# qiyueyao/Kubernetes-verification

Measured on AMD Instinct MI355X. Metric: pod-pairs/sec for reachability build + all-checks latency, 100k pods, 1/2/4/8 GPU, higher is better.
Workload: dtype u64

## Files before the change

include/kano_hip.h:

```cpp
#ifndef KANO_HIP_H
#define KANO_HIP_H

#include <stddef.h>
#include <stdint.h>

#ifdef __cplusplus
extern "C" {
#endif

typedef struct kano_ctx kano_ctx;

#define KANO_PATH_AUTO    0
#define KANO_PATH_BITWISE 1
#define KANO_PATH_MFMA    2

#define KANO_INFO_N        0
#define KANO_INFO_W        1
#define KANO_INFO_P        2
#define KANO_INFO_U        3
#define KANO_INFO_NNZ_SEL  4
#define KANO_INFO_NNZ_ALW  5
#define KANO_INFO_HEAVY    6
#define KANO_INFO_ROW0     7
#define KANO_INFO_ROW1     8
#define KANO_INFO_MAXSEL   9
#define KANO_INFO_UA      10
#define KANO_INFO_HEAVY_PATH 11
#define KANO_INFO_WORK_ITEMS 12
#define KANO_INFO_ROWS_KERNEL 13
#define KANO_INFO_ROWS_CUS 14
#define KANO_INFO_HEAVY_SEL 15
#define KANO_INFO_HEAVY_KERNEL 16
#define KANO_INFO_CLS_REUSED 17
#define KANO_INFO_NSLOTS   18

int  kano_create(int device, kano_ctx** out);
int  kano_create_lean(int device, kano_ctx** out);
void kano_destroy(kano_ctx* ctx);
const char* kano_last_error(const kano_ctx* ctx);
int  kano_set_stream(kano_ctx* ctx, void* hip_stream);

int kano_set_pods(kano_ctx* ctx, int64_t n, int32_t ncols, const int32_t* pod_val);
int kano_set_policies(kano_ctx* ctx, int64_t P,
                      const int64_t* sel_off, const int32_t* sel_col, const int32_t* sel_val,
                      const int64_t* alw_off, const int32_t* alw_col, const int32_t* alw_val);
int kano_set_shard(kano_ctx* ctx, int64_t row_begin, int64_t row_end);

int kano_build(kano_ctx* ctx, int path);
int kano_info(kano_ctx* ctx, int64_t* out );
// ... 182 lines not shown
```

kubernetes-verification_amd/csrc/kano_engine.hpp:

```cpp
#pragma once
#include <hip/hip_runtime.h>
#include <hip/hip_ext.h>

#include <algorithm>
#include <cmath>
#include <functional>
#include <cerrno>
#include <cstdint>
#include <cstdlib>
#include <cstring>
#include <string>
#include <vector>
#include <array>
#include <chrono>
#include <ctime>
#include <cstdio>
#include <dlfcn.h>
#include <link.h>
#include <thread>

#include "kano_hip.h"
#include "kano_internal.hpp"
#include "kano_prims.hpp"

// ... 26 lines not shown
  DBuf keys_d, table, smin, slot_of, flag, cid, cls, rep, mcnt, mcur, moff, mem, cval;
};

struct RowsInputs {
  DBuf wioff, wicls, soffc, slist, aloff, alist, alcoff, alc, rmoff, rmem, cmoff, cmem, ccls,
      hflag, hlist, Mc;
};

struct SideMatch {
  i64 nterms = 0;
  int NM = 0;
  bool dense = false;
  DBuf toff, tslot, tval, pmask, moff, mslot;
  DBuf table, pslot, gcnt, goff, gcur, gmem, pstart, plen, bits, bcnt, boff;
  i64 T = 0;
};

enum {
  SZ_UR = 0, SZ_UA, SZ_NNZ_SEL, SZ_NNZ_ALC, SZ_NNZ_ALW, SZ_NFLAGS, SZ_WI, SZ_HEAVY, SZ_MAXSEL,
  SZ_LIGHT, SZ_HSEL, SZ_NL, SZ_PAIRS, SZ_IDX0, SZ_IDX1, SZ_IDX2, SZ_IDX3, SZ_ERR, SZ_SLOTS = 18,
  SZ_SIGNAL = SZ_SLOTS
};

constexpr size_t ROW_STAGE_BYTES = 256 * 1024;

struct kano_ctx {
  int device = 0;
  hipStream_t stream = nullptr;
  bool own_stream = false;
  std::string err;
// ... 63 lines not shown
  bool xcd_tried = false, eng_on_xcd = false, xcd_last_ok = false;
  int side_mode = 0;
  int xcd_side = -1;
  hipStream_t stream_x = nullptr, stream2_x = nullptr, stream3x = nullptr;
  hipStream_t stream2_u = nullptr;
  hipEvent_t ev_sw = nullptr, ev_sw2 = nullptr;
  i64 rows_cu_bytes = 8ll << 30;
  int num_cus = 0, rows_cus = 0;

  ClassSet rc, cc;
  bool cls_valid = false;
  bool cls_reuse = false;
  i64 cls_U[2] = {0, 0};
  i64 cls_reused = 0;
  SideMatch sm, am;
  i64 UAW = 0, ldC = 0;
  i64 nnz_sel = 0, nnz_alc = 0, nnz_alw = 0, heavy_count = 0, wi_total = 0, nflags = 0;
  i64 heavy_sel = 0;
  i64 light_cost = 0;
  bool rows_use_alist = false;
  int max_sel = 0;
  int heavy_path = 0;
  int heavy_kernel = 0;
  int rows_kernel = 0;

  DBuf pv;
  DBuf scnt, cost, soffc, scur, slist, ecls, wicls, maxs, wicnt, wioff, hflag, hoff, hlist, sq, pfoff;
  DBuf ACT, AC, nca, acnt, alcoff, alc, aloff, alist;
  DBuf M, Mc, color, colnand, col_and, col_or_c, col_nand_c;
  DBuf scan_tmp;
// ... 157 lines not shown
struct GroupRun {
  int32_t group;
  int32_t first, len;
};
i64 group_chunks(const kano_ctx* ctx);
i64 group_run_rows(kano_ctx* ctx, i64 sel, i64 nbp, bool rows);
int group_masks_launch(kano_ctx* ctx, const int32_t* gd, i64 b0, i64 nbp, u64* maskT);
int group_rows_launch(kano_ctx* ctx, const u64* maskT, i64 b0, i64 nbp, const int32_t* order,
                      const GroupRun* runs, i64 nruns, i64 Gd, u64* counts, int32_t* row_counts);

template <typename T>
T* P_(DBuf& b) {
  return reinterpret_cast<T*>(b.p);
}

inline unsigned nblk(i64 n, i64 per = TPB) { return (unsigned)((n + per - 1) / per); }

}
```

kubernetes-verification_amd/csrc/kano_ext.hip:

```cpp
#include "kano_engine.hpp"
#include "kano_inc.hpp"
#include "kano_k8s.hpp"
#include "kano_path.hpp"
#include "kano_hops.hpp"

using namespace kano_eng;

namespace {

struct PathGeom {
  bool identity = false;
  i64 rows = 0;
  i64 Ua = 0;
  i64 KW = 0;
  i64 ldR = 0;
  const u64* base = nullptr;
  const u64* T = nullptr;
};

template <int CW>
int path_or_launch(kano_ctx* ctx, const u64* D, u64* R, u64* Dn, const PathGeom& g) {
  const i64 nch = (g.ldR + 64 * CW - 1) / (64 * CW);
  hipLaunchKernelGGL(k_path_or<CW>, dim3(nblk(g.rows * nch, TPB / 64)), dim3(TPB), 0, ctx->stream,
                     D, R, Dn, g.ldR, g.T, g.ldR, g.rows, g.KW, nch, P_<u64>(ctx->pcnt));
// ... 354 lines not shown
      return fail(ctx, -EINVAL, "kano_add_policies: allow term column out of range");
  if (ncols_x > 0 && n > 0) {
    const i64 have = ctx->inc_xcols * n, add = (i64)ncols_x * n;
    DBuf grown;
    KTRY(dalloc(ctx, grown, sizeof(int32_t) * (have + add)));
    if (have > 0)
      KCHK(hipMemcpyAsync(grown.p, ctx->xv.p, sizeof(int32_t) * have, hipMemcpyDeviceToDevice,
                          ctx->stream));
    KCHK(hipMemcpyAsync(P_<int32_t>(grown) + have, xval, sizeof(int32_t) * add,
                        hipMemcpyHostToDevice, ctx->stream));
    KTRY(sync(ctx));
    dfree(ctx->xv);
    ctx->xv = grown;
  }
  ctx->inc_xcols += ncols_x;
  if (ncols_x > 0) ctx->cls_valid = false;
  const i64 A0 = ctx->inc_A, A1 = A0 + Pn;
  if (A1 > ctx->inc_acap) {
    const i64 cap = std::max<i64>(A1, 2 * ctx->inc_acap);
    DBuf s2, a2;
    KTRY(dalloc(ctx, s2, sizeof(u64) * std::max<i64>(1, cap * W)));
    KTRY(dalloc(ctx, a2, sizeof(u64) * std::max<i64>(1, cap * W)));
    if (A0 > 0 && W > 0) {
      KCHK(hipMemcpyAsync(s2.p, ctx->asel.p, sizeof(u64) * A0 * W, hipMemcpyDeviceToDevice,
                          ctx->stream));
      KCHK(hipMemcpyAsync(a2.p, ctx->aalw.p, sizeof(u64) * A0 * W, hipMemcpyDeviceToDevice,
                          ctx->stream));
    }
    KTRY(sync(ctx));
    dfree(ctx->asel);
    dfree(ctx->aalw);
// ... 912 lines not shown
```

kubernetes-verification_amd/csrc/kano_hip.hip:

```cpp
#include "kano_engine.hpp"
#include "kano_kernels.hpp"

namespace kano_eng {

int fail(kano_ctx* ctx, int code, const std::string& msg) {
  ctx->err = msg;
  return code;
}

int settle(kano_ctx* ctx);

int dalloc(kano_ctx* ctx, DBuf& b, size_t bytes) {
  if (bytes == 0) bytes = 16;
  if (b.p && b.bytes >= bytes) return 0;
  if (b.p) {
    KTRY(settle(ctx));
    KCHK(hipFree(b.p));
    b.p = nullptr;
    b.bytes = 0;
  }
  const hipError_t e = hipMalloc(&b.p, bytes);
  if (e != hipSuccess) {
    b.p = nullptr;
    return fail(ctx, -ENOMEM, "hipMalloc(" + std::to_string(bytes) + " bytes) -> " +
// ... 248 lines not shown

void ring_bell(kano_ctx* ctx) {
  if (ctx->bell) __atomic_store_n(ctx->bell, ctx->bell_seq, __ATOMIC_SEQ_CST);
}

int unprime(kano_ctx* ctx) {
  if (!ctx->primed || ctx->priming) return 0;
  ctx->primed = false;
  ring_bell(ctx);
  ctx->gate_forced = ctx->bell_seq;
  KCHK(hipStreamSynchronize(ctx->stream));
  KCHK(hipStreamSynchronize(ctx->stream2));
  std::swap(ctx->sizes, ctx->sizes_alt);
  swap_rows_ptrs(ctx, !ctx->prime_kept);
  ctx->alist_valid = ctx->prime_alist_valid;
  return 0;
}

int sync(kano_ctx* ctx) {
  KTRY(unprime(ctx));
  KCHK(hipStreamSynchronize(ctx->stream));
  return 0;
}

int settle(kano_ctx* ctx) {
  KTRY(unprime(ctx));
  if (!ctx->async_pending) return 0;
  ctx->async_pending = false;
  KCHK(hipSetDevice(ctx->device));
  KCHK(hipStreamSynchronize(ctx->stream3));
// ... 270 lines not shown
  return 0;
}

int match_alloc(kano_ctx* ctx, SideMatch& sx, ClassSet& cs, FillBatch& fb) {
  const i64 P = ctx->P, U = cs.U;
  KTRY(dalloc(ctx, sx.pstart, sizeof(i64) * std::max<i64>(1, P)));
  KTRY(dalloc(ctx, sx.plen, sizeof(int32_t) * std::max<i64>(1, P)));
  if (P == 0) return 0;
  if (U == 0) {
    KTRY(fb.add(sx.pstart, sizeof(i64) * P, 0u));
    KTRY(fb.add(sx.plen, sizeof(int32_t) * P, 0u));
    return 0;
  }
  if (sx.dense) return 0;
  const int NM = sx.NM;
  sx.T = table_size(U);
  const i64 NT = std::max<i64>(1, (i64)NM * sx.T);
  KTRY(dalloc(ctx, sx.table, sizeof(int32_t) * NT));
  KTRY(dalloc(ctx, sx.pslot, sizeof(int32_t) * std::max<i64>(1, (i64)NM * U)));
  KTRY(dalloc(ctx, sx.gcnt, sizeof(int32_t) * NT));
  KTRY(dalloc(ctx, sx.gcur, sizeof(int32_t) * std::max<i64>(1, (i64)NM * U)));
  KTRY(dalloc(ctx, sx.goff, sizeof(int32_t) * (NT + 1)));
  KTRY(dalloc(ctx, sx.gmem, sizeof(int32_t) * ((i64)NM * U + U)));
  if (NM > 0) {
    KTRY(fb.add(sx.table, sizeof(int32_t) * NT, 0xffffffffu));
    KTRY(fb.add(sx.gcnt, sizeof(int32_t) * NT, 0u));
  }
  return 0;
}

// ... 5 lines not shown
  a.mslot = P_<int32_t>(sx.mslot);
  a.table = P_<int32_t>(sx.table);
  a.T = sx.T;
  a.pslot = P_<int32_t>(sx.pslot);
  a.gcnt = P_<int32_t>(sx.gcnt);
  a.goff = P_<int32_t>(sx.goff);
  a.gcur = P_<int32_t>(sx.gcur);
  a.gmem = P_<int32_t>(sx.gmem);
  a.toff = P_<i64>(sx.toff);
  a.tval = P_<int32_t>(sx.tval);
  a.pmask = P_<int32_t>(sx.pmask);
  a.pstart = P_<i64>(sx.pstart);
  a.plen = P_<int32_t>(sx.plen);
  a.NM = sx.NM;
  a.live = (ctx->P > 0 && cs.U > 0 && !sx.dense) ? 1 : 0;
  a.ctab = P_<u64>(cs.table);
  a.ctmask = (uint32_t)(table_size(ctx->n) - 1);
  a.csmin = P_<int32_t>(cs.smin);
  a.cpb = cls_pod_bits(ctx, cs);
  a.ccid = P_<int32_t>(cs.cid);
  a.cm0 = cs.m0;
  a.kbits = P_<int32_t>(cs.keys_d) + cs.KS;
  a.KS = cs.KS;
  return a;
}

int match_dense(kano_ctx* ctx, SideMatch& sx, ClassSet& cs);

int match_both(kano_ctx* ctx) {
  JoinPair pr{{join_side(ctx, ctx->am, ctx->cc), join_side(ctx, ctx->sm, ctx->rc)}};
  const JoinSide &a0 = pr.s[0], &a1 = pr.s[1];
  const i64 maxU = std::max(a0.live ? a0.U : 0, a1.live ? a1.U : 0);
  const unsigned rows_i = (a0.live ? a0.NM : 0) + (a1.live ? a1.NM : 0);
  const unsigned rows_f = (a0.live ? a0.NM + 1 : 0) + (a1.live ? a1.NM + 1 : 0);
  if (rows_i > 0) {
    hipLaunchKernelGGL(k_join_insert, dim3(nblk(maxU), rows_i), dim3(TPB), 0, ctx->stream, pr);
    KLAUNCH();
    ScanBatch sb(ctx);
    for (int q = 0; q < 2; ++q) {
      SideMatch& sx = q ? ctx->sm : ctx->am;
      if (pr.s[q].live && sx.NM > 0)
        KTRY(sb.add(P_<int32_t>(sx.gcnt), (i64)sx.NM * sx.T, P_<int32_t>(sx.goff)));
    }
    KTRY(sb.run());
  }
  if (rows_f > 0) {
    const unsigned nbf = nblk(maxU), nbm = nblk(ctx->P);
    hipLaunchKernelGGL(k_join_fill_match, dim3(std::max(nbf, nbm), rows_f + 2), dim3(TPB), 0,
                       ctx->stream, ctx->P, pr, (int)rows_f, nbf, nbm);
    KLAUNCH();
  }
  if (ctx->P > 0 && ctx->cc.U > 0 && ctx->am.dense) KTRY(match_dense(ctx, ctx->am, ctx->cc));
  if (ctx->P > 0 && ctx->rc.U > 0 && ctx->sm.dense) KTRY(match_dense(ctx, ctx->sm, ctx->rc));
  return 0;
}

int match_dense(kano_ctx* ctx, SideMatch& sx, ClassSet& cs) {
  const i64 P = ctx->P, U = cs.U;
  const i64 UW = (U + 63) / 64, ld = std::max<i64>(2, (UW + 1) & ~(i64)1);
  KTRY(dalloc(ctx, sx.bits, sizeof(u64) * P * ld));
  KTRY(dalloc(ctx, sx.boff, sizeof(i64) * (P + 1)));
  hipLaunchKernelGGL(k_class_eval, dim3(nblk(U), (unsigned)ctx->PB), dim3(TPB), 0, ctx->stream,
// ... 864 lines not shown
  a.colnand = P_<u64>(ctx->colnand);
  hipLaunchKernelGGL(k_rows<TPB>, dim3((unsigned)rl, (unsigned)((ldM + cww - 1) / cww)),
                     dim3(TPB), sizeof(u64) * cww, ctx->stream, a);
  KLAUNCH();
  KTRY(sync(ctx));
  ctx->cols_valid = true;
  return 0;
}

struct CrossPlan {
  bool on = false;
  const int32_t* gdev = nullptr;
  int32_t G = 0;
  bool key_lds = false;
  i64 knb = 0, kslots = 0;
};

int cross_setup(kano_ctx* ctx, const int32_t* gid, int32_t ngroups, CrossPlan& cp,
                hipStream_t st = nullptr) {
  const i64 n = ctx->n, W = ctx->W, ldM = ctx->ldM;
  KTRY(dalloc(ctx, ctx->gid, sizeof(int32_t) * std::max<i64>(1, n)));
  KTRY(dalloc(ctx, ctx->cross, sizeof(u64) * ldM));
  KTRY(dalloc(ctx, ctx->sizes, sizeof(u64) * SZ_SLOTS));
  cp.on = false;
  if (n == 0 || rows_local(ctx) == 0 || W == 0) return 0;
  int32_t G = ngroups;
  cp.gdev = P_<int32_t>(ctx->gid);
  if (!gid) {
    if (ctx->groups_n != n) return fail(ctx, -EINVAL, "crosscheck: no stored groups for these pods");
    G = ctx->groups_G;
// ... 5 lines not shown
        if (gid[i] < 0) return fail(ctx, -EINVAL, "kano_crosscheck: negative group id");
        G = std::max(G, gid[i] + 1);
      }
    }
    KCHK(hipMemcpyAsync(ctx->gid.p, gid, sizeof(int32_t) * n, hipMemcpyHostToDevice,
                        st ? st : ctx->stream));
  }
  cp.G = G;
  cp.on = true;
  return 0;
}

int cross_prepare(kano_ctx* ctx, const int32_t* gid, int32_t ngroups, CrossPlan& cp,
                  FillBatch& fb, bool setup_done = false) {
  const i64 ldM = ctx->ldM;
  if (!setup_done) KTRY(cross_setup(ctx, gid, ngroups, cp, fb.st));
  int32_t* err = reinterpret_cast<int32_t*>(P_<u64>(ctx->sizes) + SZ_ERR);
  KTRY(fb.add_raw(err, sizeof(u64), 0u));
  KTRY(fb.add(ctx->cross, sizeof(u64) * ldM, 0u));
  if (!cp.on) return 0;
  const int32_t G = cp.G;
  if (ctx->rows_dirty) return 0;
  const i64 U = ctx->rc.U, ldC = ctx->ldC;
  KTRY(dalloc(ctx, ctx->gmin, sizeof(int32_t) * std::max<i64>(1, U)));
  KTRY(dalloc(ctx, ctx->gmax, sizeof(int32_t) * std::max<i64>(1, U)));
  KTRY(dalloc(ctx, ctx->R, sizeof(u64) * std::max<i64>(1, (i64)G * ldC)));
  KTRY(dalloc(ctx, ctx->ckey, sizeof(int32_t) * std::max<i64>(1, U)));
  KTRY(dalloc(ctx, ctx->corder, sizeof(int32_t) * std::max<i64>(1, U)));
  cp.key_lds = (i64)G + 1 <= KEY_LDS_MAX;
  cp.knb = std::max<i64>(1, nblk(U, (i64)TPB * KEY_ITEMS));
  cp.kslots = cp.key_lds ? ((i64)G + 1) * cp.knb : (i64)G + 1;
  KTRY(dalloc(ctx, ctx->kcnt, sizeof(int32_t) * 2 * ((i64)G + 1) + sizeof(int32_t) * cp.kslots));
  KTRY(dalloc(ctx, ctx->koff, sizeof(int32_t) * (cp.kslots + 1)));
  KTRY(dalloc(ctx, ctx->multi, sizeof(u64) * ldC));
  KTRY(dalloc(ctx, ctx->A1, sizeof(u64) * ldC));
  KTRY(dalloc(ctx, ctx->A2, sizeof(u64) * ldC));
  KTRY(fb.add(ctx->gmin, sizeof(int32_t) * U, 0x7fffffffu));
  KTRY(fb.add(ctx->gmax, sizeof(int32_t) * U, 0xffffffffu));
  KTRY(fb.add(ctx->R, sizeof(u64) * (i64)G * ldC, 0u));
  for (DBuf* b : {&ctx->multi, &ctx->A1, &ctx->A2}) KTRY(fb.add(*b, sizeof(u64) * ldC, 0u));
  KTRY(fb.add(ctx->kcnt, sizeof(int32_t) * 2 * ((i64)G + 1), 0u));
  return 0;
}

KeySort cross_sort(kano_ctx* ctx, const CrossPlan& cp) {
  KeySort k{};
  k.U = ctx->rc.U;
  k.nb = cp.knb;
  k.mcnt = P_<int32_t>(ctx->rc.mcnt);
  k.gmin = P_<int32_t>(ctx->gmin);
  k.gmax = P_<int32_t>(ctx->gmax);
  k.G = cp.G;
  k.ckey = P_<int32_t>(ctx->ckey);
  k.hist = P_<int32_t>(ctx->kcnt) + 2 * ((i64)cp.G + 1);
  k.hoff = P_<int32_t>(ctx->koff);
  k.order = P_<int32_t>(ctx->corder);
// ... 572 lines not shown
  if (s) {
    ctx->stream = (hipStream_t)s;
  } else {
    KCHK(hipStreamCreateWithFlags(&ctx->stream, hipStreamNonBlocking));
    ctx->own_stream = true;
  }
  return 0;
}

int kano_set_pods(kano_ctx* ctx, int64_t n, int32_t ncols, const int32_t* pod_val) {
  if (!ctx) return -EINVAL;
  if (n < 0 || ncols < 0 || n >= (int64_t)INT32_MAX / 2 || (n * ncols > 0 && !pod_val))
    return fail(ctx, -EINVAL, "kano_set_pods: bad arguments");
  KCHK(hipSetDevice(ctx->device));
  KTRY(settle(ctx));
  ctx->cls_valid = false;
  ctx->n = n;
  ctx->W = (n + 63) / 64;
  ctx->ldM = std::max<i64>(LD_ALIGN, (ctx->W + LD_ALIGN - 1) / LD_ALIGN * LD_ALIGN);
  ctx->ncols = ncols;
  ctx->colbits.assign(ncols, 1);
  for (int32_t c = 0; c < ncols; ++c) {
    int32_t mx = 0, mn = 0;
    const int32_t* col = pod_val + (i64)c * n;
    for (i64 i = 0; i < n; ++i) {
      mx = std::max(mx, col[i] + 3);
      mn = std::min(mn, col[i] + 3);
    }
    int b = 1;
    while (b < 31 && (1 << b) <= mx) ++b;
    ctx->colbits[c] = mn < 0 ? 64 : b;
// ... 6 lines not shown
  ctx->r1 = n;
  ctx->have_pods = true;
  ctx->have_pols = false;
  ctx->built = false;
  return sync(ctx);
}

int kano_set_expressions(kano_ctx* ctx, int32_t E, const int32_t* col, const int32_t* op,
                         const int64_t* off, const int32_t* vals) {
  if (!ctx) return -EINVAL;
  if (!ctx->have_pods) return fail(ctx, -EINVAL, "kano_set_expressions before kano_set_pods");
  if (E < 0 || (E > 0 && (!col || !op || !off))) return fail(ctx, -EINVAL, "kano_set_expressions");
  if (E == 0) return 0;
  KCHK(hipSetDevice(ctx->device));
  KTRY(settle(ctx));
  ctx->cls_valid = false;
  const i64 n = ctx->n, nc = ctx->ncols;
  for (int32_t e = 0; e < E; ++e) {
    if (col[e] >= nc || op[e] < 0 || op[e] > 3 || off[e + 1] < off[e])
      return fail(ctx, -EINVAL, "kano_set_expressions: bad requirement");
    for (i64 k = off[e] + 1; k < off[e + 1]; ++k)
      if (vals[k - 1] >= vals[k]) return fail(ctx, -EINVAL, "kano_set_expressions: unsorted set");
  }
  DBuf grown;
  KTRY(dalloc(ctx, grown, sizeof(int32_t) * std::max<i64>(1, n * (nc + E))));
  if (n * nc > 0)
    KCHK(hipMemcpyAsync(grown.p, ctx->pv.p, sizeof(int32_t) * n * nc, hipMemcpyDeviceToDevice,
                        ctx->stream));
  const i64 nv = off[E];
  std::vector<uint8_t> h(sizeof(int32_t) * 2 * E + sizeof(i64) * (E + 1) +
                         sizeof(int32_t) * std::max<i64>(1, nv) + 16);
// ... 40 lines not shown
  for (int32_t c = 0; c < ctx->ncols; ++c)
    if (slot[c] == 0) {
      slot[c] = (int32_t)cs.keys.size();
      cs.keys.push_back(c);
    }
  const bool same_keys = cs.keys == keys_before;
  cs.KS = (int)cs.keys.size();
  std::vector<int32_t> kd(cs.keys);
  int tb = 0;
  for (int32_t c : cs.keys) {
    kd.push_back(ctx->colbits[c]);
    tb += ctx->colbits[c];
  }
  cs.packed = (tb <= 63 && ctx->cls_packed) ? 1 : 0;
  cs.tbits = tb;
  if (!same_keys || cs.packed != packed_before || cs.tbits != tbits_before) ctx->cls_valid = false;
  KTRY(dalloc(ctx, cs.keys_d, sizeof(int32_t) * std::max<size_t>(1, kd.size())));
  if (cs.KS > 0)
    KCHK(hipMemcpy(cs.keys_d.p, kd.data(), sizeof(int32_t) * kd.size(), hipMemcpyHostToDevice));
  std::vector<i64> toff(P + 1, 0);
  std::vector<int32_t> tslot, tval, pmask(std::max<i64>(1, P), -1), moff(1, 0), mslot;
  std::vector<std::vector<int32_t>> masks;
  std::vector<std::pair<int32_t, int32_t>> terms;
  tslot.reserve(nt);
  tval.reserve(nt);
  for (i64 p = 0; p < P; ++p) {
    terms.clear();
    for (i64 t = off[p]; t < off[p + 1]; ++t) terms.emplace_back(slot[col[t]], val[t]);
    std::sort(terms.begin(), terms.end());
    bool contradict = false;
    std::vector<int32_t> sl;
// ... 57 lines not shown
        if ((int)masks[m].size() == cs.KS) f = (int)m;
      if (f >= 0) {
        for (i64 p = 0; p < P; ++p) {
          if (pmask[p] == f) pmask[p] = -3;
          else if (pmask[p] > f) --pmask[p];
        }
        masks.erase(masks.begin() + f);
        sx.NM = (int)masks.size();
      }
    }
    for (auto& m : masks) {
      mslot.insert(mslot.end(), m.begin(), m.end());
      moff.push_back((int32_t)mslot.size());
    }
  }
  KTRY(dalloc(ctx, sx.toff, sizeof(i64) * (P + 1)));
  KTRY(dalloc(ctx, sx.tslot, sizeof(int32_t) * std::max<size_t>(1, tslot.size())));
  KTRY(dalloc(ctx, sx.tval, sizeof(int32_t) * std::max<size_t>(1, tval.size())));
  KTRY(dalloc(ctx, sx.pmask, sizeof(int32_t) * std::max<i64>(1, P)));
  KTRY(dalloc(ctx, sx.moff, sizeof(int32_t) * moff.size()));
  KTRY(dalloc(ctx, sx.mslot, sizeof(int32_t) * std::max<size_t>(1, mslot.size())));
  KCHK(hipMemcpyAsync(sx.toff.p, toff.data(), sizeof(i64) * (P + 1), hipMemcpyHostToDevice,
                      ctx->stream));
  if (!tslot.empty()) {
    KCHK(hipMemcpyAsync(sx.tslot.p, tslot.data(), sizeof(int32_t) * tslot.size(),
                        hipMemcpyHostToDevice, ctx->stream));
    KCHK(hipMemcpyAsync(sx.tval.p, tval.data(), sizeof(int32_t) * tval.size(),
                        hipMemcpyHostToDevice, ctx->stream));
  }
  if (P > 0)
// ... 17 lines not shown
  KTRY(settle(ctx));
  ctx->P = P;
  ctx->PB = (P + 63) / 64;
  KTRY(prepare_side(ctx, P, sel_off, sel_col, sel_val, ctx->rc, ctx->sm));
  KTRY(prepare_side(ctx, P, alw_off, alw_col, alw_val, ctx->cc, ctx->am));
  ctx->have_pols = true;
  ctx->built = false;
  return 0;
}

int kano_set_shard(kano_ctx* ctx, int64_t row_begin, int64_t row_end) {
  if (!ctx) return -EINVAL;
  if (!ctx->have_pods || row_begin < 0 || row_end < row_begin || row_end > ctx->n)
    return fail(ctx, -EINVAL, "kano_set_shard: bad row range");
  KTRY(settle(ctx));
  if (row_begin != ctx->r0 || row_end != ctx->r1) ctx->cls_valid = false;
  ctx->r0 = row_begin;
  ctx->r1 = row_end;
  ctx->built = false;
  return 0;
}

}

namespace {
using ExtraFills = std::function<int(FillBatch&)>;
int sel_place_early(kano_ctx* ctx) {
  ctx->sel_early_cap = -1;
  const i64 U = ctx->rc.U, P = ctx->P;
  if (U == 0 || P == 0 || !ctx->slist.p || !ctx->ecls.p) return 0;
  const i64 cap = (i64)(std::min(ctx->slist.bytes, ctx->ecls.bytes) / sizeof(int32_t));
// ... 11 lines not shown
  return 0;
}

int build_impl(kano_ctx* ctx, int path, bool rows_now, bool defer_cols = false,
               const ExtraFills& extra = ExtraFills(), const ExtraFills& pre_fill = ExtraFills(),
               const PreRun& pre_run = PreRun()) {
  if (!ctx) return -EINVAL;
  const bool consume = ctx->primed && ctx->consume_prime;
  ctx->consume_prime = false;
  if (!consume) KTRY(unprime(ctx));
  if (!ctx->have_pods || !ctx->have_pols) return fail(ctx, -EINVAL, "kano_build: inputs not set");
  if (path < 0 || path > 2) return fail(ctx, -EINVAL, "kano_build: unknown path");
  KCHK(hipSetDevice(ctx->device));
  ctx->cls_reuse = consume ? ctx->prime_kept : ctx->cls_valid;
  ctx->cls_valid = false;
  ctx->built = false;
  ctx->rows_deferred = false;
  ctx->lists_mode = false;
  ctx->rows_timed = false;
  ctx->rows_dirty = false;
  ctx->cols_valid = false;
  ctx->shadow_total = -1;
  ctx->conflict_total = -1;
  ctx->sig_armed = 0;
  ctx->sel_early_cap = -1;
  ctx->shg_prefilled = false;
  const i64 rl = rows_local(ctx);
  if (!ctx->defer_alloc)
    KTRY(dalloc(ctx, ctx->M, sizeof(u64) * std::max<i64>(1, rl * ctx->ldM)));
  KTRY(dalloc(ctx, ctx->color, sizeof(u64) * ctx->ldM));
// ... 3 lines not shown
  KTRY(mirror_begin(ctx));
  KTRY(do_back_pre(ctx, pre_fill, pre_run));
  KTRY(sel_place_early(ctx));
  KTRY(read_sizes(ctx));
  KTRY(stage_mark(ctx, 3, ctx->stream));
  ctx->cols_deferred = defer_cols;
  KTRY(do_back(ctx, path, extra));
  if (!defer_cols) KTRY(do_rows(ctx));
  if (rows_now) KTRY(launch_rows(ctx));
  KTRY(stage_mark(ctx, 4, ctx->stream));
  ctx->cols_valid = true;
  ctx->built = true;
  ctx->cls_valid = true;
  if (ctx->cls_reuse) ++ctx->cls_reused;
  ctx->cls_reuse = false;
  ctx->inc_A = 0;
  ctx->inc_xcols = 0;
  ctx->dead.assign((size_t)ctx->P, 0);
  ctx->user_edited = false;
  return 0;
}

}

extern "C" {

int kano_build(kano_ctx* ctx, int path) { return build_impl(ctx, path, true); }

int kano_build_classes(kano_ctx* ctx, int path) {
  if (!ctx) return -EINVAL;
// ... 13 lines not shown
  out[KANO_INFO_U] = ctx->rc.U;
  out[KANO_INFO_NNZ_SEL] = ctx->nnz_sel;
  out[KANO_INFO_NNZ_ALW] = ctx->nnz_alw;
  out[KANO_INFO_HEAVY] = ctx->heavy_count;
  out[KANO_INFO_ROW0] = ctx->r0;
  out[KANO_INFO_ROW1] = ctx->r1;
  out[KANO_INFO_MAXSEL] = ctx->max_sel;
  out[KANO_INFO_UA] = ctx->cc.U;
  out[KANO_INFO_HEAVY_PATH] = ctx->heavy_path;
  out[KANO_INFO_ROWS_CUS] = ctx->rows_cus;
  out[KANO_INFO_HEAVY_SEL] = ctx->heavy_sel;
  out[KANO_INFO_HEAVY_KERNEL] = ctx->heavy_kernel;
  out[KANO_INFO_WORK_ITEMS] = ctx->wi_total;
  out[KANO_INFO_ROWS_KERNEL] = ctx->rows_kernel;
  out[KANO_INFO_CLS_REUSED] = ctx->cls_reused;
  return 0;
}

int kano_col_checks(kano_ctx* ctx, uint64_t* col_and, uint64_t* col_or) {
  KTRY(ensure_matrix(ctx));
  if (!ctx->cols_valid) KTRY(recompute_cols(ctx));
  const i64 W = ctx->W;
  if (W == 0) return sync(ctx);
  KTRY(dalloc(ctx, ctx->col_and, sizeof(u64) * W));
  hipLaunchKernelGGL(k_col_final, dim3(nblk(W)), dim3(TPB), 0, ctx->stream,
                     P_<u64>(ctx->colnand), W, ctx->n, P_<u64>(ctx->col_and));
  KLAUNCH();
  if (col_and)
    KCHK(hipMemcpyAsync(col_and, ctx->col_and.p, sizeof(u64) * W, hipMemcpyDeviceToHost,
                        ctx->stream));
// ... 454 lines not shown

namespace {
int lists_setup(kano_ctx* ctx, const char* what, int64_t n_lists, int64_t nbits, int64_t P,
                const int64_t* soff, const int32_t* slist, const uint64_t* allow_rows) {
  if (!ctx) return -EINVAL;
  if (n_lists < 0 || nbits < 0 || P < 0 || !soff || n_lists >= (int64_t)INT32_MAX / 2)
    return fail(ctx, -EINVAL, std::string(what) + ": bad arguments");
  KCHK(hipSetDevice(ctx->device));
  KTRY(settle(ctx));
  const i64 nnz = soff[n_lists];
  for (i64 e = 0; e < nnz; ++e)
    if (slist[e] < 0 || slist[e] >= P)
      return fail(ctx, -ERANGE, std::string(what) + ": policy index out of range");
  ctx->conflict_total = -1;
  ctx->built = false;
  ctx->cls_valid = false;
  ctx->lists_mode = true;
  ctx->n = nbits;
  ctx->W = (nbits + 63) / 64;
  ctx->ldM = std::max<i64>(2, (ctx->W + 1) & ~(i64)1);
  ctx->P = P;
  ctx->PB = (P + 63) / 64;
  ctx->r0 = 0;
  ctx->r1 = n_lists;
  ctx->nnz_sel = nnz;
  ctx->rc.U = n_lists;
  ctx->cc.U = nbits;
  ctx->UAW = ctx->W;
  ctx->ldC = ctx->ldM;
  const i64 U = n_lists;
  KTRY(dalloc(ctx, ctx->soffc, sizeof(i64) * (U + 1)));
// ... 559 lines not shown
}

int verify_front(kano_ctx* ctx, int path, const int32_t* gid, int32_t ngroups, int64_t sys_row,
                 bool want_shadow, u64* words_dev, bool count_only = false) {
  ctx->vs_count_only = want_shadow && count_only;
  ctx->consume_prime = ctx->primed;
  if (ctx->async_pending && !ctx->primed) KTRY(swap_rows_inputs(ctx));
  const bool stored = !gid && ngroups == KANO_STORED_GROUPS;
  const bool want_cross = gid || stored;
  CrossPlan cp;
  ShadowPlan sp;
  auto pre_fill = [&](FillBatch& fb) -> int {
    return want_cross ? cross_prepare(ctx, gid, ngroups, cp, fb) : 0;
  };
  auto pre_run = [&](hipStream_t st) -> int {
    if (!want_cross || !cp.on) return 0;
    ScanBatch sb(ctx, st != nullptr);
    KTRY(cross_stage_a(ctx, cp, sb, st));
    KTRY(sb.run());
    return cross_stage_b1(ctx, cp, st);
  };
  auto extra = [&](FillBatch& fb) -> int {
    return want_shadow ? shadow_prepare(ctx, sp, fb) : 0;
  };
  ctx->vs_open = false;
  ctx->fork_pending = false;
  ctx->tail_compacted = false;
  bool fork_marked = false;
  const bool side_sh = want_shadow && !count_only;
  if (want_shadow) {
    ctx->fork_hook = [&](bool marked) -> int {
// ... 120 lines not shown
    if (q != hipErrorNotReady) KCHK(q);
    __builtin_ia32_pause();
    if ((spin & 0xff) == 0 && clk::now() - t0 > std::chrono::seconds(1)) {
      KCHK(hipEventSynchronize(e));
      return 0;
    }
  }
}

int prime_next(kano_ctx* ctx) {
  if (ctx->primed || !ctx->bell || ctx->stage_timing) return 0;
  KTRY(dalloc(ctx, ctx->sizes_alt, sizeof(u64) * SZ_SLOTS));
  ctx->prime_alist_valid = ctx->alist_valid;
  ctx->prime_kept = ctx->cls_valid;
  ctx->cls_reuse = ctx->cls_valid;
  KTRY(swap_rows_inputs(ctx));
  std::swap(ctx->sizes, ctx->sizes_alt);
  ctx->primed = true;
  ctx->priming = true;
  const u64 armed = ctx->sig_armed, waiting = ctx->sig_wait;
  if (!ctx->gate_wait.p) {
    KTRY(dalloc(ctx, ctx->gate_wait, sizeof(u64) * GATE_RING));
    KCHK(hipMemsetAsync(ctx->gate_wait.p, 0, sizeof(u64) * GATE_RING, ctx->stream));
  }
  hipLaunchKernelGGL(k_gate, dim3(1), dim3(64), 0, ctx->stream, (const u64*)ctx->bell_dev,
                     ++ctx->bell_seq, ctx->gate_ticks, P_<u64>(ctx->gate_wait));
  int rc = hipGetLastError() == hipSuccess ? 0 : fail(ctx, -EIO, "k_gate launch failed");
  if (!rc) {
    ctx->sig_armed = 0;
    rc = front_a(ctx);
// ... 71 lines not shown
    KTRY(rc);
  }
  if (async && ctx->pipeline) KTRY(prime_next(ctx));
  part(12);
  const auto tw0 = clk::now();
  KTRY(spin_event(ctx, ctx->ev_tail));
  ctx->ht[18] += std::chrono::duration<double, std::micro>(clk::now() - tw0).count();
  part(14);
  ctx->sig_wait = 0;
  constexpr int NS = SZ_ERR - SZ_NL + 1;
  i64 v[NS];
  for (int q = 0; q < NS; ++q) v[q] = (i64)((volatile u64*)ctx->gmirror)[SZ_NL + q];
  if (ctx->vs_cross_on && (v[SZ_ERR - SZ_NL] & 0xffffffff)) {
    (void)settle(ctx);
    (void)sync(ctx);
    return fail(ctx, -EINVAL, "kano_verify: a group id lies outside [0, ngroups)");
  }
  for (int r = 0; r < 4; ++r) counts[r] = v[SZ_IDX0 - SZ_NL + r];
  if (!ctx->vs_have_sys) counts[3] = -1;
  if (want_shadow) {
    const i64 total = v[SZ_PAIRS - SZ_NL];
    *shadow_count = total;
    ctx->shadow_total = pairs_mode ? total : -1;
    if (pairs_mode && total > out_cap) {
      KTRY(unprime(ctx));
      KTRY(dalloc(ctx, ctx->out, sizeof(int2) * (total + total / 4)));
      if (rl > 0) {
        hipLaunchKernelGGL(k_shadow_emit, dim3(nblk(rl)), dim3(TPB), 0, st,
                           P_<int32_t>(ctx->rc.cls), ctx->r0, ctx->r1, P_<i64>(ctx->loff),
                           P_<int2>(ctx->L), P_<i64>(ctx->poff), P_<int2>(ctx->out), total,
// ... 83 lines not shown
  };
  const bool signalled = ctx->sig_armed != 0;
  KTRY(mirror_begin(ctx));
  hipEvent_t tail_ev = signalled ? nullptr : ctx->ev_sizes;
  const bool async = may_async && ctx->async_rows;
  if (!tail_ev) {
    KCHK(hipEventRecord(ctx->ev_sizes, ctx->stream));
    tail_ev = ctx->ev_sizes;
  }
  part(12);
  i64 v[NS];
  KTRY(mirror_wait(ctx, SZ_NL, NS, v));
  tmark = clk::now();
  if (ctx->vs_cross_on && (v[SZ_ERR - SZ_NL] & 0xffffffff)) {
    (void)sync(ctx);
    return fail(ctx, -EINVAL, "kano_verify: a group id lies outside [0, ngroups)");
  }
  i64 nidx = 0;
  for (int r = 0; r < 4; ++r) {
    counts[r] = v[SZ_IDX0 - SZ_NL + r];
    nidx += counts[r];
  }
  if (!ctx->vs_have_sys) counts[3] = -1;
  hipStream_t cs = ctx->stream2;
  KCHK(hipStreamWaitEvent(cs, tail_ev, 0));
  i64 total = 0;
  if (want_shadow) {
    total = v[SZ_PAIRS - SZ_NL];
    if (shadow_cap >= 0) {
      KTRY(shadow_back(ctx, v[0], total, cs));
// ... 234 lines not shown
  ctx->vs_have_sys = have_sys;
  ctx->vs_sys_on = sys_on;
  ctx->vs_rows = false;
  ctx->vs_nb = nb;
  ctx->vs_rl = rows_local(ctx);
  return 0;
}

int kano_set_groups(kano_ctx* ctx, const int32_t* gid, int32_t ngroups) {
  if (!ctx) return -EINVAL;
  if (!ctx->have_pods) return fail(ctx, -EINVAL, "kano_set_groups before kano_set_pods");
  const i64 n = ctx->n;
  if (n > 0 && !gid) return fail(ctx, -EINVAL, "kano_set_groups: gid is NULL");
  KCHK(hipSetDevice(ctx->device));
  KTRY(settle(ctx));
  int32_t G = 0;
  for (i64 i = 0; i < n; ++i) {
    if (gid[i] < 0) return fail(ctx, -EINVAL, "kano_set_groups: negative group id");
    G = std::max(G, gid[i] + 1);
  }
  if (ngroups > 0 && ngroups < G) return fail(ctx, -EINVAL, "kano_set_groups: id >= ngroups");
  if (ngroups > 0) G = ngroups;
  KTRY(dalloc(ctx, ctx->gids, sizeof(int32_t) * std::max<i64>(1, n)));
  if (n > 0)
    KCHK(hipMemcpyAsync(ctx->gids.p, gid, sizeof(int32_t) * n, hipMemcpyHostToDevice,
                        ctx->stream));
  KTRY(sync(ctx));
  ctx->groups_n = n;
  ctx->groups_G = G;
  return 0;
// ... 105 lines not shown
```

kubernetes-verification_amd/csrc/kano_kernels.hpp:

```cpp
#pragma once
#include "kano_prims.hpp"

namespace kano {

struct ClsSide {
  const int32_t* keys;
  int KS;
  int packed;
  int pbits;
  uint32_t tmask;
  int32_t* table;
  int32_t* slot_of;
  int32_t* smin;
  int32_t* flag;
  const int32_t* cid;
  int32_t* cls;
  int32_t* rep;
  int32_t* mcnt;
  int32_t* mcur;
  const int32_t* moff;
  int32_t* mem;
  int32_t* cval;
  i64 m0, m1, U;
};
// ... 444 lines not shown
  const int32_t* mslot;
  int32_t* table;
  i64 T;
  int32_t* pslot;
  int32_t* gcnt;
  const int32_t* goff;
  int32_t* gcur;
  int32_t* gmem;
  const i64* toff;
  const int32_t* tval;
  const int32_t* pmask;
  i64* pstart;
  int32_t* plen;
  int NM;
  int live;
  const u64* ctab;
  uint32_t ctmask;
  const int32_t* csmin;
  int cpb;
  const int32_t* ccid;
  i64 cm0;
  const int32_t* kbits;
  int KS;
};
struct JoinPair {
  JoinSide s[2];
};

__device__ __forceinline__ int join_row(const JoinPair& pr, int y, int extra, int* m) {
  const int r0 = pr.s[0].live ? pr.s[0].NM + extra : 0;
  if (y < r0) { *m = y; return 0; }
  *m = y - r0;
  return 1;
}

__global__ __launch_bounds__(TPB) void k_join_insert(JoinPair pr) {
  int m;
  const JoinSide a = join_row(pr, blockIdx.y, 0, &m) ? pr.s[1] : pr.s[0];
  const i64 c = (i64)blockIdx.x * TPB + threadIdx.x;
  const bool act = c < a.U;
  uint32_t s = 0;
  if (act) {
    const int32_t* sl = a.mslot + a.moff[m];
    const int ns = a.moff[m + 1] - a.moff[m];
    int32_t* tab = a.table + (i64)m * a.T;
// ... 3117 lines not shown
```

kubernetes-verification_amd/kano/_native.py:

```python
from __future__ import annotations

import ctypes
import os
from ctypes import POINTER, c_double, c_float, c_int, c_int32, c_int64, c_uint8, c_uint64, c_void_p

_HERE = os.path.dirname(os.path.abspath(__file__))
LIB_PATH = os.environ.get(
    "KANO_HIP_LIB", os.path.join(os.path.dirname(_HERE), "csrc", "libkano_hip.so"))

SIGNATURES = {
    "kano_create": (c_int, [c_int, POINTER(c_void_p)]),
    "kano_create_lean": (c_int, [c_int, POINTER(c_void_p)]),
    "kano_destroy": (None, [c_void_p]),
    "kano_last_error": (ctypes.c_char_p, [c_void_p]),
    "kano_set_stream": (c_int, [c_void_p, c_void_p]),
    "kano_set_pods": (c_int, [c_void_p, c_int64, c_int32, c_void_p]),
    "kano_set_policies": (c_int, [c_void_p, c_int64, c_void_p, c_void_p, c_void_p,
                                  c_void_p, c_void_p, c_void_p]),
    "kano_set_shard": (c_int, [c_void_p, c_int64, c_int64]),
    "kano_build": (c_int, [c_void_p, c_int]),
    "kano_info": (c_int, [c_void_p, c_void_p]),
    "kano_col_checks": (c_int, [c_void_p, c_void_p, c_void_p]),
    "kano_col_flags_dev": (c_int, [c_void_p, c_void_p]),
    "kano_crosscheck": (c_int, [c_void_p, c_void_p, c_void_p]),
# ... 85 lines not shown
    "kano_group_checks": (c_int, [c_void_p, c_void_p, c_int32, c_int64, c_void_p, c_void_p]),
    "kano_group_upload": (c_int, [c_void_p, c_int64, c_int32, c_void_p, c_int32, c_void_p,
                                  c_void_p, c_void_p, c_void_p, c_int64, c_void_p, c_void_p,
                                  c_void_p, c_void_p, c_void_p, c_void_p, c_void_p]),
    "kano_group_build": (c_int, [c_void_p, c_int]),
    "kano_group_set_groups": (c_int, [c_void_p, c_void_p, c_int32]),
    "kano_group_add_policies": (c_int, [c_void_p, c_int64, c_int32, c_void_p] + [c_void_p] * 6 +
                                [POINTER(c_int64)]),
    "kano_group_remove_policies": (c_int, [c_void_p, c_int64, c_void_p]),
    "kano_group_path": (c_int, [c_void_p, c_void_p, c_int, c_int, c_void_p]),
    "kano_group_exchange_timing": (c_int, [c_void_p, c_int, c_void_p, c_int]),
    "kano_host_alloc": (c_int, [ctypes.c_size_t, POINTER(c_void_p)]),
    "kano_host_free": (None, [c_void_p]),
}

INFO_SLOTS = 18
INFO = dict(N=0, W=1, P=2, U=3, NNZ_SEL=4, NNZ_ALW=5, HEAVY=6, ROW0=7, ROW1=8, MAXSEL=9,
            UA=10, HEAVY_PATH=11, WORK_ITEMS=12, ROWS_KERNEL=13, ROWS_CUS=14,
            HEAVY_SEL=15, HEAVY_KERNEL=16, CLS_REUSED=17)
PATHS = {"auto": 0, "bitwise": 1, "mfma": 2}
STORED_GROUPS = -1
GROUP_LEAN, GROUP_RCCL, GROUP_COPY = 1, 2, 4


class KanoNativeError(RuntimeError):
    pass


_lib = None


def load(path: str = LIB_PATH) -> ctypes.CDLL:
    global _lib
    if _lib is not None:
# ... 34 lines not shown
```

Baseline: 33230 billion.

## Reuse join hash groups and cross-group tables across rebuilds when inputs unchanged

Extends class reuse across builds. The join hash tables are kept when the match-slot layout (moff/mslot) is unchanged, and the cross-check gmin/gmax/kcnt stage is kept when stored group ids and the group count are unchanged. Every input mutation path now invalidates these caches, and new info counters report how often they were reused. This skips join insert, scan and cross stage-A work on repeated builds, at the cost of host copies of slot vectors and more complex invalidation logic that could serve stale results.

```diff
diff --git a/include/kano_hip.h b/include/kano_hip.h
--- a/include/kano_hip.h
+++ b/include/kano_hip.h
@@ -32,7 +32,9 @@
 #define KANO_INFO_HEAVY_SEL 15
 #define KANO_INFO_HEAVY_KERNEL 16
 #define KANO_INFO_CLS_REUSED 17
-#define KANO_INFO_NSLOTS   18
+#define KANO_INFO_JOIN_REUSED 18
+#define KANO_INFO_CROSS_REUSED 19
+#define KANO_INFO_NSLOTS   20
 
 int  kano_create(int device, kano_ctx** out);
 int  kano_create_lean(int device, kano_ctx** out);
diff --git a/kubernetes-verification_amd/csrc/kano_engine.hpp b/kubernetes-verification_amd/csrc/kano_engine.hpp
--- a/kubernetes-verification_amd/csrc/kano_engine.hpp
+++ b/kubernetes-verification_amd/csrc/kano_engine.hpp
@@ -64,6 +64,10 @@
   DBuf toff, tslot, tval, pmask, moff, mslot;
   DBuf table, pslot, gcnt, goff, gcur, gmem, pstart, plen, bits, bcnt, boff;
   i64 T = 0;
+  bool groups_valid = false;
+  bool groups_reuse = false;
+  bool prime_groups = false;
+  std::vector<int32_t> h_moff, h_mslot;
 };
 
 enum {
@@ -157,6 +161,14 @@
   i64 cls_U[2] = {0, 0};
   i64 cls_reused = 0;
   SideMatch sm, am;
+  i64 join_reused = 0;
+  bool cross_valid = false;
+  bool cross_reuse = false;
+  bool cross_seen = false;
+  bool cross_made = false;
+  bool cross_taken = false;
+  int32_t cross_keep_G = 0;
+  i64 cross_reused = 0;
   i64 UAW = 0, ldC = 0;
   i64 nnz_sel = 0, nnz_alc = 0, nnz_alw = 0, heavy_count = 0, wi_total = 0, nflags = 0;
   i64 heavy_sel = 0;
@@ -344,6 +356,13 @@
   return reinterpret_cast<T*>(b.p);
 }
 
+inline void drop_classes(kano_ctx* ctx) {
+  ctx->cls_valid = false;
+  ctx->sm.groups_valid = false;
+  ctx->am.groups_valid = false;
+  ctx->cross_valid = false;
+}
+
 inline unsigned nblk(i64 n, i64 per = TPB) { return (unsigned)((n + per - 1) / per); }
 
 }
diff --git a/kubernetes-verification_amd/csrc/kano_ext.hip b/kubernetes-verification_amd/csrc/kano_ext.hip
--- a/kubernetes-verification_amd/csrc/kano_ext.hip
+++ b/kubernetes-verification_amd/csrc/kano_ext.hip
@@ -392,7 +392,7 @@
     ctx->xv = grown;
   }
   ctx->inc_xcols += ncols_x;
-  if (ncols_x > 0) ctx->cls_valid = false;
+  if (ncols_x > 0) drop_classes(ctx);
   const i64 A0 = ctx->inc_A, A1 = A0 + Pn;
   if (A1 > ctx->inc_acap) {
     const i64 cap = std::max<i64>(A1, 2 * ctx->inc_acap);
diff --git a/kubernetes-verification_amd/csrc/kano_hip.hip b/kubernetes-verification_amd/csrc/kano_hip.hip
--- a/kubernetes-verification_amd/csrc/kano_hip.hip
+++ b/kubernetes-verification_amd/csrc/kano_hip.hip
@@ -286,6 +286,8 @@
   std::swap(ctx->sizes, ctx->sizes_alt);
   swap_rows_ptrs(ctx, !ctx->prime_kept);
   ctx->alist_valid = ctx->prime_alist_valid;
+  for (SideMatch* sx : {&ctx->sm, &ctx->am})
+    if (!sx->prime_groups) sx->groups_valid = false;
   return 0;
 }
 
@@ -586,6 +588,7 @@
   }
   if (sx.dense) return 0;
   const int NM = sx.NM;
+  if (sx.groups_reuse) return 0;
   sx.T = table_size(U);
   const i64 NT = std::max<i64>(1, (i64)NM * sx.T);
   KTRY(dalloc(ctx, sx.table, sizeof(int32_t) * NT));
@@ -621,6 +624,7 @@
   a.plen = P_<int32_t>(sx.plen);
   a.NM = sx.NM;
   a.live = (ctx->P > 0 && cs.U > 0 && !sx.dense) ? 1 : 0;
+  a.kept = (a.live && sx.groups_reuse) ? 1 : 0;
   a.ctab = P_<u64>(cs.table);
   a.ctmask = (uint32_t)(table_size(ctx->n) - 1);
   a.csmin = P_<int32_t>(cs.smin);
@@ -637,22 +641,23 @@
 int match_both(kano_ctx* ctx) {
   JoinPair pr{{join_side(ctx, ctx->am, ctx->cc), join_side(ctx, ctx->sm, ctx->rc)}};
   const JoinSide &a0 = pr.s[0], &a1 = pr.s[1];
-  const i64 maxU = std::max(a0.live ? a0.U : 0, a1.live ? a1.U : 0);
-  const unsigned rows_i = (a0.live ? a0.NM : 0) + (a1.live ? a1.NM : 0);
-  const unsigned rows_f = (a0.live ? a0.NM + 1 : 0) + (a1.live ? a1.NM + 1 : 0);
+  const bool b0 = a0.live && !a0.kept, b1 = a1.live && !a1.kept;
+  const i64 maxU = std::max(b0 ? a0.U : 0, b1 ? a1.U : 0);
+  const unsigned rows_i = (b0 ? a0.NM : 0) + (b1 ? a1.NM : 0);
+  const unsigned rows_f = (b0 ? a0.NM + 1 : 0) + (b1 ? a1.NM + 1 : 0);
   if (rows_i > 0) {
     hipLaunchKernelGGL(k_join_insert, dim3(nblk(maxU), rows_i), dim3(TPB), 0, ctx->stream, pr);
     KLAUNCH();
     ScanBatch sb(ctx);
     for (int q = 0; q < 2; ++q) {
       SideMatch& sx = q ? ctx->sm : ctx->am;
-      if (pr.s[q].live && sx.NM > 0)
+      if (pr.s[q].live && !pr.s[q].kept && sx.NM > 0)
         KTRY(sb.add(P_<int32_t>(sx.gcnt), (i64)sx.NM * sx.T, P_<int32_t>(sx.goff)));
     }
     KTRY(sb.run());
   }
-  if (rows_f > 0) {
-    const unsigned nbf = nblk(maxU), nbm = nblk(ctx->P);
+  if (a0.live || a1.live) {
+    const unsigned nbf = rows_f > 0 ? nblk(maxU) : 0, nbm = nblk(ctx->P);
     hipLaunchKernelGGL(k_join_fill_match, dim3(std::max(nbf, nbm), rows_f + 2), dim3(TPB), 0,
                        ctx->stream, ctx->P, pr, (int)rows_f, nbf, nbm);
     KLAUNCH();
@@ -1547,6 +1552,7 @@
   int32_t G = 0;
   bool key_lds = false;
   i64 knb = 0, kslots = 0;
+  bool kept = false;
 };
 
 int cross_setup(kano_ctx* ctx, const int32_t* gid, int32_t ngroups, CrossPlan& cp,
@@ -1582,6 +1588,11 @@
 int cross_prepare(kano_ctx* ctx, const int32_t* gid, int32_t ngroups, CrossPlan& cp,
                   FillBatch& fb, bool setup_done = false) {
   const i64 ldM = ctx->ldM;
+  const bool offered = ctx->cross_reuse;
+  ctx->cross_reuse = false;
+  ctx->cross_valid = false;
+  ctx->cross_made = false;
+  ctx->cross_seen = true;
   if (!setup_done) KTRY(cross_setup(ctx, gid, ngroups, cp, fb.st));
   int32_t* err = reinterpret_cast<int32_t*>(P_<u64>(ctx->sizes) + SZ_ERR);
   KTRY(fb.add_raw(err, sizeof(u64), 0u));
@@ -1603,11 +1614,19 @@
   KTRY(dalloc(ctx, ctx->multi, sizeof(u64) * ldC));
   KTRY(dalloc(ctx, ctx->A1, sizeof(u64) * ldC));
   KTRY(dalloc(ctx, ctx->A2, sizeof(u64) * ldC));
-  KTRY(fb.add(ctx->gmin, sizeof(int32_t) * U, 0x7fffffffu));
-  KTRY(fb.add(ctx->gmax, sizeof(int32_t) * U, 0xffffffffu));
+  const bool stored = cp.gdev == P_<int32_t>(ctx->gids);
+  cp.kept = offered && stored && G == ctx->cross_keep_G;
+  ctx->cross_made = stored;
+  ctx->cross_keep_G = G;
+  ctx->cross_taken = cp.kept;
+  if (!cp.kept) {
+    KTRY(fb.add(ctx->gmin, sizeof(int32_t) * U, 0x7fffffffu));
+    KTRY(fb.add(ctx->gmax, sizeof(int32_t) * U, 0xffffffffu));
+  }
   KTRY(fb.add(ctx->R, sizeof(u64) * (i64)G * ldC, 0u));
   for (DBuf* b : {&ctx->multi, &ctx->A1, &ctx->A2}) KTRY(fb.add(*b, sizeof(u64) * ldC, 0u));
-  KTRY(fb.add(ctx->kcnt, sizeof(int32_t) * 2 * ((i64)G + 1), 0u));
+  if (!cp.kept)
+    KTRY(fb.add(ctx->kcnt, sizeof(int32_t) * 2 * ((i64)G + 1), 0u));
   return 0;
 }
 
@@ -2210,7 +2229,7 @@
     return fail(ctx, -EINVAL, "kano_set_pods: bad arguments");
   KCHK(hipSetDevice(ctx->device));
   KTRY(settle(ctx));
-  ctx->cls_valid = false;
+  drop_classes(ctx);
   ctx->n = n;
   ctx->W = (n + 63) / 64;
   ctx->ldM = std::max<i64>(LD_ALIGN, (ctx->W + LD_ALIGN - 1) / LD_ALIGN * LD_ALIGN);
@@ -2247,7 +2266,7 @@
   if (E == 0) return 0;
   KCHK(hipSetDevice(ctx->device));
   KTRY(settle(ctx));
-  ctx->cls_valid = false;
+  drop_classes(ctx);
   const i64 n = ctx->n, nc = ctx->ncols;
   for (int32_t e = 0; e < E; ++e) {
     if (col[e] >= nc || op[e] < 0 || op[e] > 3 || off[e + 1] < off[e])
@@ -2318,7 +2337,7 @@
   }
   cs.packed = (tb <= 63 && ctx->cls_packed) ? 1 : 0;
   cs.tbits = tb;
-  if (!same_keys || cs.packed != packed_before || cs.tbits != tbits_before) ctx->cls_valid = false;
+  if (!same_keys || cs.packed != packed_before || cs.tbits != tbits_before) drop_classes(ctx);
   KTRY(dalloc(ctx, cs.keys_d, sizeof(int32_t) * std::max<size_t>(1, kd.size())));
   if (cs.KS > 0)
     KCHK(hipMemcpy(cs.keys_d.p, kd.data(), sizeof(int32_t) * kd.size(), hipMemcpyHostToDevice));
@@ -2406,6 +2425,9 @@
       moff.push_back((int32_t)mslot.size());
     }
   }
+  if (sx.dense || moff != sx.h_moff || mslot != sx.h_mslot) sx.groups_valid = false;
+  sx.h_moff = moff;
+  sx.h_mslot = mslot;
   KTRY(dalloc(ctx, sx.toff, sizeof(i64) * (P + 1)));
   KTRY(dalloc(ctx, sx.tslot, sizeof(int32_t) * std::max<size_t>(1, tslot.size())));
   KTRY(dalloc(ctx, sx.tval, sizeof(int32_t) * std::max<size_t>(1, tval.size())));
@@ -2453,7 +2475,7 @@
   if (!ctx->have_pods || row_begin < 0 || row_end < row_begin || row_end > ctx->n)
     return fail(ctx, -EINVAL, "kano_set_shard: bad row range");
   KTRY(settle(ctx));
-  if (row_begin != ctx->r0 || row_end != ctx->r1) ctx->cls_valid = false;
+  if (row_begin != ctx->r0 || row_end != ctx->r1) drop_classes(ctx);
   ctx->r0 = row_begin;
   ctx->r1 = row_end;
   ctx->built = false;
@@ -2495,6 +2517,14 @@
   KCHK(hipSetDevice(ctx->device));
   ctx->cls_reuse = consume ? ctx->prime_kept : ctx->cls_valid;
   ctx->cls_valid = false;
+  for (SideMatch* sx : {&ctx->sm, &ctx->am}) {
+    sx->groups_reuse = consume ? sx->prime_groups : (ctx->cls_reuse && sx->groups_valid);
+    sx->groups_valid = false;
+  }
+  const bool cross_before = ctx->cls_reuse && ctx->cross_valid;
+  ctx->cross_reuse = cross_before;
+  ctx->cross_valid = false;
+  ctx->cross_seen = ctx->cross_made = ctx->cross_taken = false;
   ctx->built = false;
   ctx->rows_deferred = false;
   ctx->lists_mode = false;
@@ -2528,6 +2558,13 @@
   ctx->cls_valid = true;
   if (ctx->cls_reuse) ++ctx->cls_reused;
   ctx->cls_reuse = false;
+  if (ctx->sm.groups_reuse || ctx->am.groups_reuse) ++ctx->join_reused;
+  ctx->sm.groups_valid = ctx->P > 0 && ctx->rc.U > 0 && !ctx->sm.dense && ctx->sm.NM > 0;
+  ctx->am.groups_valid = ctx->P > 0 && ctx->cc.U > 0 && !ctx->am.dense && ctx->am.NM > 0;
+  ctx->sm.groups_reuse = ctx->am.groups_reuse = false;
+  ctx->cross_valid = ctx->cross_seen ? ctx->cross_made : cross_before;
+  if (ctx->cross_taken) ++ctx->cross_reused;
+  ctx->cross_reuse = ctx->cross_seen = ctx->cross_made = ctx->cross_taken = false;
   ctx->inc_A = 0;
   ctx->inc_xcols = 0;
   ctx->dead.assign((size_t)ctx->P, 0);
@@ -2571,6 +2608,8 @@
   out[KANO_INFO_WORK_ITEMS] = ctx->wi_total;
   out[KANO_INFO_ROWS_KERNEL] = ctx->rows_kernel;
   out[KANO_INFO_CLS_REUSED] = ctx->cls_reused;
+  out[KANO_INFO_JOIN_REUSED] = ctx->join_reused;
+  out[KANO_INFO_CROSS_REUSED] = ctx->cross_reused;
   return 0;
 }
 
@@ -3055,7 +3094,7 @@
       return fail(ctx, -ERANGE, std::string(what) + ": policy index out of range");
   ctx->conflict_total = -1;
   ctx->built = false;
-  ctx->cls_valid = false;
+  drop_classes(ctx);
   ctx->lists_mode = true;
   ctx->n = nbits;
   ctx->W = (nbits + 63) / 64;
@@ -3645,7 +3684,7 @@
     return want_cross ? cross_prepare(ctx, gid, ngroups, cp, fb) : 0;
   };
   auto pre_run = [&](hipStream_t st) -> int {
-    if (!want_cross || !cp.on) return 0;
+    if (!want_cross || !cp.on || cp.kept) return 0;
     ScanBatch sb(ctx, st != nullptr);
     KTRY(cross_stage_a(ctx, cp, sb, st));
     KTRY(sb.run());
@@ -3796,6 +3835,8 @@
   ctx->prime_alist_valid = ctx->alist_valid;
   ctx->prime_kept = ctx->cls_valid;
   ctx->cls_reuse = ctx->cls_valid;
+  for (SideMatch* sx : {&ctx->sm, &ctx->am})
+    sx->groups_reuse = sx->prime_groups = ctx->cls_valid && sx->groups_valid;
   KTRY(swap_rows_inputs(ctx));
   std::swap(ctx->sizes, ctx->sizes_alt);
   ctx->primed = true;
@@ -3897,6 +3938,7 @@
   if (ctx->vs_cross_on && (v[SZ_ERR - SZ_NL] & 0xffffffff)) {
     (void)settle(ctx);
     (void)sync(ctx);
+    drop_classes(ctx);
     return fail(ctx, -EINVAL, "kano_verify: a group id lies outside [0, ngroups)");
   }
   for (int r = 0; r < 4; ++r) counts[r] = v[SZ_IDX0 - SZ_NL + r];
@@ -4010,6 +4052,7 @@
   tmark = clk::now();
   if (ctx->vs_cross_on && (v[SZ_ERR - SZ_NL] & 0xffffffff)) {
     (void)sync(ctx);
+    drop_classes(ctx);
     return fail(ctx, -EINVAL, "kano_verify: a group id lies outside [0, ngroups)");
   }
   i64 nidx = 0;
@@ -4274,6 +4317,7 @@
   if (n > 0 && !gid) return fail(ctx, -EINVAL, "kano_set_groups: gid is NULL");
   KCHK(hipSetDevice(ctx->device));
   KTRY(settle(ctx));
+  ctx->cross_valid = false;
   int32_t G = 0;
   for (i64 i = 0; i < n; ++i) {
     if (gid[i] < 0) return fail(ctx, -EINVAL, "kano_set_groups: negative group id");
diff --git a/kubernetes-verification_amd/csrc/kano_kernels.hpp b/kubernetes-verification_amd/csrc/kano_kernels.hpp
--- a/kubernetes-verification_amd/csrc/kano_kernels.hpp
+++ b/kubernetes-verification_amd/csrc/kano_kernels.hpp
@@ -482,6 +482,7 @@
   int32_t* plen;
   int NM;
   int live;
+  int kept;
   const u64* ctab;
   uint32_t ctmask;
   const int32_t* csmin;
@@ -496,7 +497,7 @@
 };
 
 __device__ __forceinline__ int join_row(const JoinPair& pr, int y, int extra, int* m) {
-  const int r0 = pr.s[0].live ? pr.s[0].NM + extra : 0;
+  const int r0 = pr.s[0].live && !pr.s[0].kept ? pr.s[0].NM + extra : 0;
   if (y < r0) { *m = y; return 0; }
   *m = y - r0;
   return 1;
diff --git a/kubernetes-verification_amd/kano/_native.py b/kubernetes-verification_amd/kano/_native.py
--- a/kubernetes-verification_amd/kano/_native.py
+++ b/kubernetes-verification_amd/kano/_native.py
@@ -123,10 +123,11 @@
     "kano_host_free": (None, [c_void_p]),
 }
 
-INFO_SLOTS = 18
+INFO_SLOTS = 20
 INFO = dict(N=0, W=1, P=2, U=3, NNZ_SEL=4, NNZ_ALW=5, HEAVY=6, ROW0=7, ROW1=8, MAXSEL=9,
             UA=10, HEAVY_PATH=11, WORK_ITEMS=12, ROWS_KERNEL=13, ROWS_CUS=14,
-            HEAVY_SEL=15, HEAVY_KERNEL=16, CLS_REUSED=17)
+            HEAVY_SEL=15, HEAVY_KERNEL=16, CLS_REUSED=17, JOIN_REUSED=18,
+            CROSS_REUSED=19)
 PATHS = {"auto": 0, "bitwise": 1, "mfma": 2}
 STORED_GROUPS = -1
 GROUP_LEAN, GROUP_RCCL, GROUP_COPY = 1, 2, 4
```

Measured after the change: 33680 billion (median of 6 runs). About the same (+1.4%).
